# tbpaolini/PyJpegDecoder

Measured on AMD Instinct MI355X. Metric: megapixels/sec decoded (1080p 4:2:0 baseline batch), higher is better.
Workload: dtype f32; 1 GPU; 1024 x 1920x1080 4:2:0 baseline JPEG per GPU, q85, DRI=120 (one MCU row, 68 segments/image), on-GPU Huffman + dequant/IDCT/upsample/RGB (BASELINE configs[2]); images_per_gpu=1024, images_all_gpus=1024, distinct_images_per_gpu=256, layout=xmajor, restart_segmentation=host, entropy_bytes_per_image=667743

## Files before the change

pyjpegdecoder_amd/csrc/fused.hip:

```cpp
#include <stdio.h>
#include <string.h>

#include <algorithm>
#include <type_traits>
#include <vector>

#include "mijpeg_internal.h"
#include "lanes13_walk.h"
#include "reconstruct_fast_strips.h"

#pragma clang fp contract(off)

namespace mj {

namespace {

constexpr int kFusedLds = 160 * 1024;
constexpr int kFusedCtrl = 384;
constexpr int kFusedBitmap = 128;
constexpr int kFusedThreads = 1024;

struct FusedArgs {
    lanes13::Args L;
    ReconArgs R;
    const int64_t *job_prefix;
    int64_t total_jobs;
    int32_t jobs_per_image;
    int32_t n_prod, n_cons;
    int32_t ipw, n_pass, n_virt;
    int32_t spi;
    int32_t ri;
    int32_t n_images;
    int32_t pieces, piece_mcus, mcus_per_row, mcu_rows;
    int32_t col_pieces, piece_rows;
    int32_t simd_split;
    int32_t newest;
    uint32_t *x_counter;
    uint32_t *x_progress;
    const int32_t *x_holder;
    uint32_t *x_left;
    int32_t x_patience;
};

typedef uint32_t __attribute__((address_space(3))) *lds_word;
typedef uint32_t __attribute__((address_space(3))) *lds_word_t;

constexpr unsigned long long kFusedGuardTicks = 200000000ull;
__device__ __forceinline__ bool guard_expired(unsigned long long t0) { return __builtin_amdgcn_s_memrealtime() - t0 > kFusedGuardTicks; }

struct JobGeo {
    uint32_t ri, mpr, mcv, spi;
    uint32_t pieces, piece_mcus;
    uint32_t col_pieces, piece_rows;
};

template <bool BY_ROWS>
struct FusedSource {
    static constexpr bool kSingleJobs = true;
    uint32_t ctrl;
    uint32_t n_tickets;
    uint32_t v0, n_pass, ipp, n_images;
    uint32_t jobs_per_image, lpw;
    JobGeo g;
    int32_t *status;
    int lane;
    uint32_t newest, wpi, n_prod_w, pref;
    __device__ __forceinline__ uint32_t ctl_word(uint32_t addr) const {
        return (uint32_t)__builtin_amdgcn_readfirstlane((int)*(volatile uint32_t __attribute__((address_space(3))) *)(uintptr_t)addr);
    }
    __device__ __forceinline__ uint32_t claim() const {
        const uint32_t ih = images_in(0);
        for (;;) {
            const bool all_done = ctl_word(ctrl + 4u) >= n_prod_w;
            for (uint32_t jj = 0; jj < ih; ++jj) {
                const uint32_t j = pref + jj < ih ? pref + jj : pref + jj - ih;
                uint32_t r = g.mpr;
                if (!all_done) {
                    const uint32_t w0 = (j * g.spi) / lpw, w1 = (j * g.spi + g.spi - 1u) / lpw;
                    for (uint32_t w = w0; w <= w1; ++w) r = min(r, ctl_word(ctrl + 8u + 4u * w));
                }
                while (r > 0u) {
                    const uint32_t w = (r - 1u) >> 5, hi = r - (w << 5);
                    const uint32_t addr = ctrl + (uint32_t)kFusedBitmap + 4u * (j * wpi + w);
                    const uint32_t avail = ~ctl_word(addr) & (hi >= 32u ? 0xFFFFFFFFu : (1u << hi) - 1u);
                    if (avail == 0u) { r = w << 5; continue; }
                    const uint32_t b = 31u - (uint32_t)__builtin_clz(avail);
                    uint32_t old = 0;
                    if (lane == 0) old = __hip_atomic_fetch_or((lds_word_t)(uintptr_t)addr, 1u << b, __ATOMIC_RELAXED, __HIP_MEMORY_SCOPE_WORKGROUP);
                    old = (uint32_t)__builtin_amdgcn_readfirstlane((int)old);
                    if (!(old & (1u << b))) return (v0 * ipp + j) * jobs_per_image + (w << 5) + b;
                }
            }
            if (all_done) return ~0u;
            __builtin_amdgcn_s_sleep(8);
        }
    }
    __device__ __forceinline__ uint32_t images_in(uint32_t pass) const {
        const uint32_t lo = (v0 + pass) * ipp;
        return lo >= n_images ? 0u : min(ipp, n_images - lo);
    }
    __device__ __forceinline__ uint32_t draw() const {
        uint32_t t = 0;
        if (lane == 0) t = __hip_atomic_fetch_add((lds_word)(uintptr_t)ctrl, 1u, __ATOMIC_RELAXED, __HIP_MEMORY_SCOPE_WORKGROUP);
        return t;
    }
    __device__ __forceinline__ uint32_t take(uint32_t t) const { return (uint32_t)__builtin_amdgcn_readfirstlane((int)t); }
    __device__ __forceinline__ uint32_t first_job(uint32_t ticket) const {
        if constexpr (!BY_ROWS) { if (newest) return claim(); }
        uint32_t pass = 0, ih = images_in(0);
        for (; pass + 1 < n_pass; ++pass) {
            const uint32_t tp = ih * jobs_per_image;
            if (ticket < tp) break;
            ticket -= tp;
            ih = images_in(pass + 1);
        }
        const uint32_t img0 = (v0 + pass) * ipp;
        if constexpr (BY_ROWS) {
            const uint32_t rows = ih * g.mcv, pc = ticket / rows, rr = ticket - pc * rows, j = rr / g.mcv, row = rr - j * g.mcv;
            return (img0 + j) * jobs_per_image + row * g.pieces + pc;
        } else {
            const uint32_t m = ticket / ih, j = ticket - m * ih;
            return (img0 + j) * jobs_per_image + m;
        }
    }
    __device__ __forceinline__ uint32_t end_job(uint32_t ticket, uint32_t) const { return newest ? 0u : first_job(ticket) + 1u; }
    __device__ __forceinline__ uint32_t word(uint32_t j, uint32_t s) const {
        return *(volatile uint32_t __attribute__((address_space(3))) *)(uintptr_t)(ctrl + 8u + 4u * ((j * g.spi + s) / lpw));
    }
    __device__ __forceinline__ bool ready(uint32_t job) const {
        if (newest) return true;
        const uint32_t img = job / jobs_per_image, m = job - img * jobs_per_image, v = img / ipp, j = img - v * ipp;
        const uint32_t base = (v - v0) << kFusedPassShift;
        if constexpr (BY_ROWS) {
            const uint32_t row = m / g.pieces, pc = m - row * g.pieces, a = pc * g.piece_mcus, b = min(a + g.piece_mcus, g.mpr);
            const uint32_t g0 = row * g.mpr + a, g1 = row * g.mpr + b - 1u;
            bool ok = true;
            for (uint32_t s = g0 / g.ri; s <= g1 / g.ri; ++s) {
                const uint32_t need = min(g1, (s + 1u) * g.ri - 1u) - s * g.ri;
                ok = ok && (uint32_t)__builtin_amdgcn_readfirstlane((int)word(j, s)) > base + need;
            }
            return ok;
        }
        const uint32_t mc = m / g.col_pieces, q = m - mc * g.col_pieces, r_lo = q * g.piece_rows, r_hi = min(r_lo + g.piece_rows, g.mcv);
        if (g.ri == g.mpr) {
            const uint32_t w0 = (j * g.spi + r_lo) / lpw, w1 = (j * g.spi + r_hi - 1u) / lpw;
            uint32_t least = 0x7FFFFFFFu;
            for (uint32_t w = w0; w <= w1; ++w) {
                const uint32_t p = *(volatile uint32_t __attribute__((address_space(3))) *)(uintptr_t)(ctrl + 8u + 4u * w);
                least = min(least, p);
            }
            return (uint32_t)__builtin_amdgcn_readfirstlane((int)least) > base + mc;
        }
        bool behind = false;
        for (uint32_t r0 = r_lo; r0 < r_hi; r0 += 64u) {
            const uint32_t row = r0 + (uint32_t)lane;
            if (row < r_hi) {
                const uint32_t gi = row * g.mpr + mc, s = gi / g.ri;
                behind = behind || word(j, s) <= base + (gi - s * g.ri);
            }
        }
        return __builtin_amdgcn_ballot_w64(behind) == 0;
    }
    __device__ __forceinline__ bool wait_ready(uint32_t job) const {
        if (ready(job)) return true;
        const unsigned long long t0 = __builtin_amdgcn_s_memrealtime();
        while (!ready(job)) {
            __builtin_amdgcn_s_sleep(8);
            if (guard_expired(t0)) {
                if (lane == 0) atomicMax(status + job / jobs_per_image, MJ_ST_INTERNAL);
                break;
            }
        }
        return true;
    }
};

template <bool BY_ROWS>
struct FusedSourceX {
    static constexpr bool kSingleJobs = true;
    uint32_t *counter;
    const uint32_t *progress;
    const int32_t *holder;
    uint32_t n_tickets, n_images, jobs_per_image;
    JobGeo g;
    uint32_t *left_count, *left_list;
    uint32_t patience;
    int32_t *status;
    int lane;
    __device__ __forceinline__ uint32_t draw() const {
        uint32_t t = 0;
        if (lane == 0) t = __hip_atomic_fetch_add(counter, 1u, __ATOMIC_RELAXED, __HIP_MEMORY_SCOPE_AGENT);
        return t;
    }
    __device__ __forceinline__ uint32_t take(uint32_t t) const { return (uint32_t)__builtin_amdgcn_readfirstlane((int)t); }
    __device__ __forceinline__ uint32_t first_job(uint32_t ticket) const {
        if constexpr (BY_ROWS) {
            const uint32_t rows = n_images * g.mcv, pc = ticket / rows, rr = ticket - pc * rows, img = rr / g.mcv, row = rr - img * g.mcv;
            return img * jobs_per_image + row * g.pieces + pc;
        } else {
            const uint32_t m = ticket / n_images, img = ticket - m * n_images;
            return img * jobs_per_image + m;
        }
    }
    __device__ __forceinline__ uint32_t end_job(uint32_t ticket, uint32_t) const { return first_job(ticket) + 1u; }
    __device__ __forceinline__ uint32_t word(uint32_t img, uint32_t s) const {
        return __hip_atomic_load(progress + holder[img * g.spi + s], __ATOMIC_RELAXED, __HIP_MEMORY_SCOPE_AGENT);
    }
    __device__ __forceinline__ bool ready(uint32_t job) const {
        const uint32_t img = job / jobs_per_image, m = job - img * jobs_per_image;
        bool behind = false;
        if constexpr (BY_ROWS) {
            const uint32_t row = m / g.pieces, pc = m - row * g.pieces, a = pc * g.piece_mcus, b = min(a + g.piece_mcus, g.mpr);
// ... 3 lines not shown
            const uint32_t mc = m / g.col_pieces, q = m - mc * g.col_pieces, r_lo = q * g.piece_rows, r_hi = min(r_lo + g.piece_rows, g.mcv);
            for (uint32_t r0 = r_lo; r0 < r_hi; r0 += 64u) {
                const uint32_t row = r0 + (uint32_t)lane;
                if (row < r_hi) {
                    const uint32_t gi = row * g.mpr + mc, s = gi / g.ri;
                    behind = behind || word(img, s) <= gi - s * g.ri;
                }
            }
        }
        if (__builtin_amdgcn_ballot_w64(behind) != 0) return false;
        __builtin_amdgcn_fence(__ATOMIC_ACQUIRE, "agent");
        return true;
    }
    __device__ __forceinline__ bool wait_ready(uint32_t job) const {
        for (uint32_t spins = 0; !ready(job); ++spins) {
            __builtin_amdgcn_s_sleep(16);
            if (spins >= patience) {
                if (lane == 0) left_list[__hip_atomic_fetch_add(left_count, 1u, __ATOMIC_RELAXED, __HIP_MEMORY_SCOPE_AGENT)] = job;
                return false;
            }
        }
        return true;
    }
};

}

template <int HS, int VS, bool T, bool XWG>
__global__ __launch_bounds__(kFusedThreads) void k_fused(FusedArgs F) {
    using G = rfast::FGeo<HS, VS, 3>;
    extern __shared__ __attribute__((aligned(16))) unsigned char smem[];
    const int tid = threadIdx.x, lane = tid & 63;
    const int n_prod = F.n_prod, n_cons = F.n_cons;
    int wave = __builtin_amdgcn_readfirstlane(tid >> 6);
    if (F.simd_split) {
        const int simd = wave & 3, slot = wave >> 2, r = slot * 2 + (simd & 1);
        if (simd < 2) wave = r < n_prod ? r : n_prod + n_cons + (r - n_prod);
        else wave = r < n_cons ? n_prod + r : n_prod + n_cons + (8 - min(n_prod, 8)) + (r - n_cons);
        wave = min(wave, kFusedThreads / 64 - 1);
    }
    uint32_t *ctrl = reinterpret_cast<uint32_t *>(smem + kFusedLds - kFusedCtrl);
    float4 *wts = reinterpret_cast<float4 *>(smem + kFusedLds - kFusedCtrl - G::WTS_BYTES);
    if (tid < kFusedCtrl / 4) ctrl[tid] = 0;
    lanes13::stage<true>(F.L, smem, tid, kFusedThreads, n_prod);
    rfast::fill_weights<HS, VS, 3, T>(wts, tid, kFusedThreads);
    __syncthreads();

    typename std::conditional<XWG, FusedSourceX<T>, FusedSource<T>>::type src;
    const uint32_t ctrl_lds = lanes13::lds_addr(ctrl);
    const uint32_t v0 = (uint32_t)blockIdx.x * (uint32_t)F.n_pass;
    src.n_images = (uint32_t)F.n_images;
    src.jobs_per_image = (uint32_t)F.jobs_per_image;
    src.g = JobGeo{(uint32_t)F.ri, (uint32_t)F.mcus_per_row, (uint32_t)F.mcu_rows, (uint32_t)F.spi, (uint32_t)F.pieces, (uint32_t)F.piece_mcus,
                   (uint32_t)F.col_pieces, (uint32_t)F.piece_rows};
    if constexpr (XWG) {
        src.counter = F.x_counter; src.progress = F.x_progress; src.holder = F.x_holder;
        src.left_count = F.x_counter + 1; src.left_list = F.x_left; src.patience = (uint32_t)F.x_patience;
        src.n_tickets = src.n_images * src.jobs_per_image;
    } else {
        src.ctrl = ctrl_lds;
        src.v0 = v0; src.n_pass = (uint32_t)F.n_pass; src.ipp = (uint32_t)F.ipw;
        src.lpw = (uint32_t)F.L.lpw;
        src.newest = (uint32_t)F.newest; src.wpi = ((uint32_t)F.mcus_per_row + 31u) >> 5; src.n_prod_w = (uint32_t)n_prod;
        src.pref = (uint32_t)wave % max(1u, src.images_in(0));
        uint32_t mine = 0;
        for (uint32_t p = 0; p < src.n_pass; ++p) mine += src.images_in(p);
        src.n_tickets = mine * src.jobs_per_image;
    }
    src.lane = lane;
    src.status = F.L.status;

#ifdef MJ_DIAGNOSTIC
    unsigned long long *dbg = reinterpret_cast<unsigned long long *>(F.R.dump + (3u << 20)) + (size_t)(blockIdx.x & 1023) * 8;
    if (tid == 0) dbg[0] = __builtin_amdgcn_s_memrealtime();
#endif
    unsigned long long *clk = reinterpret_cast<unsigned long long *>(F.R.dump + kDumpClockWords);
    if (blockIdx.x == 0 && tid == 0) { clk[0] = __builtin_amdgcn_s_memtime(); clk[1] = __builtin_amdgcn_s_memrealtime(); }
    unsigned char *my_lds;
    if (wave < n_prod) {
        if constexpr (XWG) {
            lanes13::walk<2>(F.L, smem, lane, wave, n_prod, (int)blockIdx.x, (int)gridDim.x, lanes13::lds_addr(ctrl + 2 + wave));
        } else {
            for (int p = 0; p < F.n_pass && (int)v0 + p < F.n_virt; ++p)
                lanes13::walk<1>(F.L, smem, lane, wave, n_prod, (int)v0 + p, F.n_virt, lanes13::lds_addr(ctrl + 2 + wave), (uint32_t)p << kFusedPassShift);
        }
        __builtin_amdgcn_s_setprio(0);
#ifdef MJ_DIAGNOSTIC
        if (lane == 0) {
            const unsigned long long t = __builtin_amdgcn_s_memrealtime();
            atomicMin(dbg + 1, t);
            atomicMax(dbg + 2, t);
            if constexpr (!XWG) atomicMax(dbg + 4, (unsigned long long)*(volatile uint32_t __attribute__((address_space(3))) *)(uintptr_t)ctrl_lds);
        }
#endif
        if (lane == 0) __hip_atomic_fetch_add((lds_word)(uintptr_t)lanes13::lds_addr(ctrl + 1), 1u, __ATOMIC_RELEASE, __HIP_MEMORY_SCOPE_WORKGROUP);
    }
    if (wave >= n_prod && wave < n_prod + n_cons) {
        my_lds = smem + kFusedLds - kFusedCtrl - G::WTS_BYTES - (wave - n_prod + 1) * G::WAVE_BYTES;
    } else {
        {
            const unsigned long long t0 = __builtin_amdgcn_s_memrealtime();
            while ((int)*(volatile uint32_t __attribute__((address_space(3))) *)(uintptr_t)(ctrl_lds + 4u) < n_prod) {
                __builtin_amdgcn_s_sleep(16);
                if (guard_expired(t0)) return;
            }
        }
        __builtin_amdgcn_fence(__ATOMIC_ACQUIRE, "workgroup");
        const int k = wave < n_prod ? wave : wave - n_cons;
        if (k >= (int)((kFusedLds - kFusedCtrl - G::WTS_BYTES) / G::WAVE_BYTES) - n_cons) return;
        my_lds = smem + k * G::WAVE_BYTES;
    }
    rfast::strips_worker<HS, VS, 3, false, T>(F.R, F.job_prefix, F.total_jobs, F.jobs_per_image, my_lds, wts, lane, (int)blockIdx.x, wave, src);
    if (blockIdx.x == 0 && lane == 0) {
        atomicMax(clk + 2, (unsigned long long)__builtin_amdgcn_s_memtime());
        atomicMax(clk + 3, (unsigned long long)__builtin_amdgcn_s_memrealtime());
    }
#ifdef MJ_DIAGNOSTIC
    if (lane == 0) atomicMax(dbg + 3, (unsigned long long)__builtin_amdgcn_s_memrealtime());
#endif
}

#ifdef MJ_DIAGNOSTIC
void dbg_fused_report(const uint8_t *dump, int n_wg) {
    std::vector<unsigned long long> h((size_t)1024 * 8);
    (void)hipMemcpy(h.data(), dump + (3u << 20), h.size() * 8, hipMemcpyDeviceToHost);
    double first = 0, last = 0, end = 0, drawn = 0, end_max = 0;
    const int n = std::min(n_wg, 1024);
    unsigned long long t0 = ~0ull;
    for (int i = 0; i < n; ++i) t0 = std::min(t0, h[(size_t)i * 8]);
    for (int i = 0; i < n; ++i) {
        const unsigned long long *r = h.data() + (size_t)i * 8;
        first += (double)(r[1] - r[0]) * 0.01; last += (double)(r[2] - r[0]) * 0.01; end += (double)(r[3] - r[0]) * 0.01; drawn += (double)r[4];
        end_max = std::max(end_max, (double)(r[3] - t0) * 0.01);
    }
    fprintf(stderr, "[diag fused] %d workgroups; per workgroup (us from its start): first producer through %.0f, last %.0f, last wave out %.0f; tickets drawn when the "
                    "last producer was through %.0f; launch (first start to last end) %.0f us\n", n, first / n, last / n, end / n, drawn / n, end_max);
}
void dbg_fused_clear(uint8_t *dump) {
    std::vector<unsigned long long> z((size_t)1024 * 8, 0);
    for (size_t i = 0; i < 1024; ++i) z[i * 8 + 1] = ~0ull;
    (void)hipMemcpy(dump + (3u << 20), z.data(), z.size() * 8, hipMemcpyHostToDevice);
}
#endif


template <bool BY_ROWS>
struct LeftoverSource {
    static constexpr bool kSingleJobs = true;
    FusedSourceX<BY_ROWS> map;
    uint32_t *counter;
    const uint32_t *list;
    uint32_t n_left, first_undrawn, n_tickets;
    int lane;
    __device__ __forceinline__ uint32_t draw() const {
        uint32_t t = 0;
        if (lane == 0) t = __hip_atomic_fetch_add(counter, 1u, __ATOMIC_RELAXED, __HIP_MEMORY_SCOPE_AGENT);
        return t;
    }
    __device__ __forceinline__ uint32_t take(uint32_t t) const { return (uint32_t)__builtin_amdgcn_readfirstlane((int)t); }
    __device__ __forceinline__ uint32_t first_job(uint32_t ticket) const {
        return ticket < n_left ? list[ticket] : map.first_job(first_undrawn + (ticket - n_left));
    }
    __device__ __forceinline__ uint32_t end_job(uint32_t ticket, uint32_t) const { return first_job(ticket) + 1u; }
    __device__ __forceinline__ bool ready(uint32_t) const { return true; }
    __device__ __forceinline__ bool wait_ready(uint32_t) const { return true; }
};

template <int HS, int VS, bool T>
__global__ __launch_bounds__(256, 3) void k_recon_leftover(FusedArgs F) {
    using G = rfast::FGeo<HS, VS, 3>;
    extern __shared__ __attribute__((aligned(16))) unsigned char smem[];
    const uint32_t n_left = __hip_atomic_load(F.x_counter + 1, __ATOMIC_RELAXED, __HIP_MEMORY_SCOPE_AGENT);
    const uint32_t all = (uint32_t)F.n_images * (uint32_t)F.jobs_per_image;
    const uint32_t drawn = min(__hip_atomic_load(F.x_counter, __ATOMIC_RELAXED, __HIP_MEMORY_SCOPE_AGENT), all);
    if (n_left == 0 && drawn == all) return;
    const int tid = threadIdx.x, lane = tid & 63;
    const int wave = __builtin_amdgcn_readfirstlane(tid >> 6);
    if constexpr (G::SUB) {
        rfast::fill_weights<HS, VS, 3, T>(reinterpret_cast<float4 *>(smem + 4 * G::WAVE_BYTES), tid, 256);
        __syncthreads();
    }
// ... 72 lines not shown

extern "C" int mj_debug_fused_shape(int32_t cus, int32_t n_ac, int32_t n_dc, int32_t ac_slot_bytes, int32_t hmax, int32_t vmax, int32_t transposed,
                                    int32_t n_images, int32_t segments_per_image, int32_t want_consumers, int32_t out[8]) {
    if (!out) return MJ_ERR_INVALID;
    const mj::FusedShape s = mj::fused_shape(cus, n_ac * ac_slot_bytes, n_dc, hmax, vmax, transposed != 0, n_images, segments_per_image, want_consumers);
    out[0] = s.ok ? 1 : 0; out[1] = s.ipw; out[2] = s.n_prod; out[3] = s.lpw; out[4] = s.n_cons;
    out[5] = s.ok ? (int32_t)mj::lanes13::lds_bytes(s.ac_total_bytes, n_dc, s.n_prod, s.lpw, s.ring, s.dbits) : 0;
    out[6] = s.n_pass; out[7] = s.n_wg;
    return MJ_OK;
}

namespace mj {

hipError_t launch_fused(hipStream_t stream, const FusedShape &shape, const uint32_t *dstream, const int32_t *seg_bits, const DevSegment *segs,
                        int64_t n_segs, const DevImage *images, const DevHuff *huff, const uint16_t *lut11, const uint32_t *lut13,
                        int n_ac, int n_dc, uint64_t ac_slot_pk, uint64_t dc_slot_pk, uint64_t dc_tab_pk, const int ac_off[4], const int ac_bits[4],
                        int16_t *coef, int32_t *status,
                        const ReconArgs &a, int hmax, int vmax, bool transposed, int spi, int restart_interval, int mcus_per_row, int mcu_rows,
                        const int64_t *job_prefix, int64_t total_jobs, int jobs_per_image, const int32_t *by_length, const int32_t *holder,
                        uint32_t *x_words) {
    if (restart_interval < 1 || spi < 1) return hipErrorInvalidValue;
    if (!shape.ok || a.n_images < 1) return hipErrorInvalidValue;
    if (shape.xwg && (!by_length || !holder || !x_words)) return hipErrorInvalidValue;
    FusedArgs F{};
    F.L = lanes13::Args{dstream, seg_bits, segs, n_segs, images, huff, lut11, lut13, n_ac, n_dc, ac_slot_pk, dc_slot_pk, dc_tab_pk,
                        coef, status, shape.lpw, transposed ? 1 : 0, nullptr, nullptr, 0, shape.ring, shape.ac_total_bytes, shape.dbits,
                        {ac_off[0], ac_off[1], ac_off[2], ac_off[3]}, {ac_bits[0], ac_bits[1], ac_bits[2], ac_bits[3]}, shape.ipw * spi, nullptr};
    F.R = a;
    F.job_prefix = job_prefix; F.total_jobs = total_jobs; F.jobs_per_image = jobs_per_image;
    F.n_prod = shape.n_prod; F.n_cons = shape.n_cons; F.ipw = shape.ipw; F.n_pass = shape.n_pass; F.n_virt = shape.n_virt;
    F.spi = spi; F.ri = restart_interval; F.n_images = a.n_images;
    F.pieces = 1; F.piece_mcus = mcus_per_row; F.mcus_per_row = mcus_per_row; F.mcu_rows = mcu_rows;
    F.col_pieces = 1; F.piece_rows = mcu_rows;
    if (const char *e = opt("MJ_FUSED_SIMD_SPLIT")) F.simd_split = atoi(e) != 0 && shape.n_prod <= 8 && shape.n_cons <= 8;
    F.newest = !shape.xwg && !transposed && shape.n_pass == 1 && restart_interval == mcus_per_row && F.col_pieces == 1 &&
               shape.ipw * ((mcus_per_row + 31) / 32) <= (kFusedCtrl - kFusedBitmap) / 4;
    if (const char *e = opt("MJ_FUSED_ORDER")) F.newest = F.newest && !strcmp(e, "newest");
    else F.newest = 0;
    if (!transposed) {
        const int tmw = fast_tile_mcus(hmax, vmax, 3, false), spc = (mcu_rows + tmw - 1) / tmw;
        F.col_pieces = (spc + a.chunk_strips - 1) / a.chunk_strips;
        F.piece_rows = a.chunk_strips * tmw;
        if (jobs_per_image != mcus_per_row * F.col_pieces) return hipErrorInvalidValue;
    }
    if (transposed) {
        const int tmw = fast_tile_mcus(hmax, vmax, 3, true);
        int piece = 20;
        if (const char *e = opt("MJ_FUSED_PIECE")) piece = atoi(e);
        const int strips = std::max(1, piece / tmw);
        const int spc = (mcus_per_row + tmw - 1) / tmw;
        F.R.chunk_strips = strips;
        F.pieces = (spc + strips - 1) / strips;
        F.piece_mcus = strips * tmw;
        F.jobs_per_image = mcu_rows * F.pieces;
        F.total_jobs = (int64_t)a.n_images * F.jobs_per_image;
    }
    unsigned blocks = 0;
    if (shape.xwg) {
        const int64_t words = 32 + (int64_t)shape.n_wg * shape.n_prod;
        if (hipError_t e = launch_fill_words(stream, x_words, 0u, words); e != hipSuccess) return e;
        F.x_counter = x_words; F.x_progress = x_words + 32; F.x_holder = holder;
        F.x_left = x_words + 32 + (int64_t)shape.n_wg * shape.n_prod;
        F.x_patience = 2000;
        if (const char *e = opt("MJ_FUSED_PATIENCE")) F.x_patience = atoi(e);
        F.L.by_length = by_length; F.L.order_mode = 2; F.L.progress_global = F.x_progress;
        blocks = (unsigned)shape.n_wg;
    } else {
        blocks = (unsigned)shape.n_wg;
    }
    auto go = [&](auto kernel) {
        static OncePerDevice attr_once;
// ... 47 lines not shown
```

pyjpegdecoder_amd/csrc/options.hip:

```cpp
#include <string.h>
#include <stdlib.h>

#include <mutex>
#include <string>

#include "mijpeg_internal.h"

namespace mj {
namespace {
struct OptionRule { const char *name; const char *words; int lo, hi, step; };
const OptionRule kOptionRules[] = {
    {"MJ_HUFFMAN", "wave|lanes|lanes11|sync", 0, 0, 1}, {"MJ_SEG_ORDER", "blob|binned|striped", 0, 0, 1},
    {"MJ_SYNC_ROUNDS", nullptr, 0, 64, 1},   {"MJ_SYNC_CHUNK", nullptr, 256, 65536, 4}, {"MJ_SYNC_WARM", nullptr, 0, 65536, 1},
    {"MJ_PROG_BANDS", nullptr, 0, 1, 1},     {"MJ_PROG_ROWS", nullptr, 1, 4096, 1},     {"MJ_PROG_FAST", nullptr, 0, 1, 1},
    {"MJ_LANES_WAVES", nullptr, 1, 16, 1},   {"MJ_LANES_PER_WAVE", nullptr, 1, 64, 1},  {"MJ_LANES_RING", "64|128", 0, 0, 1},
    {"MJ_STAGE2_CHUNK", nullptr, 1, 4096, 1}, {"MJ_PROG_SPLIT", nullptr, 0, 3, 1},      {"MJ_PROG_PARTS", nullptr, 1, kProgSub, 1},
    {"MJ_FUSED", nullptr, 0, 1, 1},          {"MJ_FUSED_CONSUMERS", nullptr, 0, 15, 1},  {"MJ_FUSED_PATIENCE", nullptr, 0, 1000000, 1},
    {"MJ_FUSED_LUMA13", nullptr, 0, 1, 1},   {"MJ_SYNC_COUNT", "classic|resolved", 0, 0, 1}, {"MJ_SYNC_BITS", nullptr, 10, 13, 1},
    {"MJ_FUSED_ACBITS", nullptr, 10, 13, 1}, {"MJ_FUSED_PRODUCERS", nullptr, 1, 8, 1}, {"MJ_FUSED_SIMD_SPLIT", nullptr, 0, 1, 1}, {"MJ_FUSED_ORDER", "ticket|newest", 0, 0, 1},
    {"MJ_FUSED_PIECE", nullptr, 1, 4096, 1},
    {"MJ_PROG_CHUNKS", nullptr, 0, 2, 1},    {"MJ_PROG_CHUNK", nullptr, 128, 65536, 4},
};
constexpr int kNumOptions = (int)(sizeof(kOptionRules) / sizeof(kOptionRules[0]));
struct OptionTable {
    std::mutex mu;
    struct Entry { std::string value; bool set = false; };
    Entry e[kNumOptions];
};
OptionTable g_options;
bool option_value_ok(const OptionRule &r, const char *v) {
    if (r.words) {
        const size_t n = strlen(v);
        for (const char *w = r.words; *w;) {
            const char *bar = strchr(w, '|');
            const size_t len = bar ? (size_t)(bar - w) : strlen(w);
            if (len == n && !strncmp(w, v, n)) return true;
            w += len + (bar ? 1 : 0);
        }
        return false;
    }
    char *end = nullptr;
    const long x = strtol(v, &end, 10);
    return end != v && *end == 0 && x >= r.lo && x <= r.hi && x % r.step == 0;
}
}
const char *opt(const char *name) {
    thread_local std::string ring[8];
    thread_local unsigned turn = 0;
    {
        std::lock_guard<std::mutex> lk(g_options.mu);
        for (int i = 0; i < kNumOptions; ++i)
            if (!strcmp(kOptionRules[i].name, name)) {
// ... 49 lines not shown
```

pyjpegdecoder_amd/csrc/reconstruct_fast_strips.h:

```cpp
#pragma once
#include "mijpeg_internal.h"
#include "upsample_taps.h"

#pragma clang fp contract(off)

namespace mj {
namespace rfast {

#ifdef MJ_X_NTLOAD
typedef uint32_t mj_u32x4 __attribute__((ext_vector_type(4)));
__device__ __forceinline__ uint4 coef_load_nt(const uint4 *p) {
    const mj_u32x4 v = __builtin_nontemporal_load(reinterpret_cast<const mj_u32x4 *>(p));
    return make_uint4(v.x, v.y, v.z, v.w);
}
#define MJ_COEF_LOAD(p) coef_load_nt(p)
#else
#define MJ_COEF_LOAD(p) (*(p))
#endif

constexpr double kA = 0.35355339059327373;
constexpr double kC2 = 0.46193976625564337, kC6 = 0.19134171618254492;
constexpr double kC1 = 0.4903926402016152, kC3 = 0.4157348061512726, kC5 = 0.27778511650980114, kC7 = 0.09754516100806417;

__device__ __forceinline__ void idct8(const double f[8], double t[8]) {
// ... 197 lines not shown
}

static __device__ __noinline__ void block_exact(const int16_t *cblk, const uint16_t *qblk, const double *tt, int16_t *out_lds,
                                         int16_t *idct_out , bool transposed, bool chroma) {
    const int lane = threadIdx.x & 63;
    const int u = lane >> 3, v = lane & 7;
    const int src = transposed ? u * 8 + v : v * 8 + u;
    const int dn = deq(cblk[src], qblk[src]);
    const uint64_t mask = __ballot(dn != 0);
    double rsum[8];
#pragma unroll
    for (int vv = 0; vv < 8; ++vv) rsum[vv] = 0.0;
#pragma unroll 1
    for (int uu = 0; uu < 8; ++uu) {
        const uint32_t rowbits = (uint32_t)(mask >> (uu * 8)) & 0xFFu;
        if (rowbits == 0) continue;
#pragma unroll
        for (int vv = 0; vv < 8; ++vv) {
            if ((rowbits >> vv) & 1) {
                const int cc = __builtin_amdgcn_readlane(dn, uu * 8 + vv);
                const double p = (double)cc * tt[(uu * 8 + vv) * 64 + lane];
                rsum[vv] = rsum[vv] + p;
            }
        }
    }
    const double s = ((rsum[0] + rsum[1]) + (rsum[2] + rsum[3])) + ((rsum[4] + rsum[5]) + (rsum[6] + rsum[7]));
    const int raw = (int)(int16_t)(int)__builtin_rint(s), val = (int)(int16_t)(raw + 128);
    out_lds[transposed ? (lane & 7) * 8 + (lane >> 3) : lane] = (int16_t)(chroma ? raw : val);
    if (idct_out) idct_out[lane] = (int16_t)val;
}

struct TicketSource {
    static constexpr bool kSingleJobs = false;
    uint32_t *counter;
    uint32_t jpt, n_tickets, last_ticket;
    int lane;
    __device__ __forceinline__ uint32_t draw() const {
        uint32_t t = 0;
        if (lane == 0) t = __hip_atomic_fetch_add(counter, 1u, __ATOMIC_RELAXED, __HIP_MEMORY_SCOPE_AGENT);
        return t;
    }
    __device__ __forceinline__ uint32_t take(uint32_t t) const {
        const uint32_t c = (uint32_t)__builtin_amdgcn_readfirstlane((int)t);
        if (c == last_ticket && lane == 0) __hip_atomic_store(counter, 0u, __ATOMIC_RELAXED, __HIP_MEMORY_SCOPE_AGENT);
        return c;
    }
    __device__ __forceinline__ uint32_t first_job(uint32_t ticket) const { return ticket * jpt; }
    __device__ __forceinline__ uint32_t end_job(uint32_t ticket, uint32_t n_jobs) const { return min(n_jobs, (ticket + 1) * jpt); }
    __device__ __forceinline__ bool ready(uint32_t) const { return true; }
    __device__ __forceinline__ bool wait_ready(uint32_t) const { return true; }
};

template <int HS, int VS, int NC, bool T>
__device__ __forceinline__ void fill_weights(float4 *wt, int tid, int nthreads) {
    using G = FGeo<HS, VS, NC>;
    if constexpr (G::SUB) {
        constexpr float D = (float)kDen<HS, VS>;
        for (int i = tid; i < G::MW * G::MH; i += nthreads) {
            const uint32_t w = corner_weights<HS, VS, T>(i / G::MH, i % G::MH);
            wt[(i / G::MH) * G::WTS_ROW + (i % G::MH)] = make_float4((float)(w & 255) / D, (float)((w >> 8) & 255) / D, (float)((w >> 16) & 255) / D,
                                                                   (float)(w >> 24) / D);
        }
    }
}

template <int HS, int VS, int NC, bool SEAMS, bool T, class Src>
__device__ __forceinline__ void strips_worker(const ReconArgs &a, const int64_t *__restrict__ job_prefix, const int64_t total_jobs, const int jobs_per_image,
                                              unsigned char *wave_lds, const float4 *s_wts, const int lane, const int dump_slot, const int wave_in_wg, Src &src) {
    using G = FGeo<HS, VS, NC>;
    int16_t *s_strip = reinterpret_cast<int16_t *>(wave_lds);
    double *scr = reinterpret_cast<double *>(wave_lds + G::STRIP_BYTES) + (lane >> 3) * 72;
    float *scrf = reinterpret_cast<float *>(wave_lds + G::STRIP_BYTES) + (lane >> 3) * 124;
    uint16_t *s_qt = reinterpret_cast<uint16_t *>(wave_lds + G::STRIP_BYTES + G::SCR_BYTES);
    const int grp = lane >> 3, j = lane & 7;

    const int px = lane / G::TML, pk0 = lane % G::TML;

    struct Job {
        const DevImage *im;
        const int16_t *cfirst;
        int row_elems;
        int mcu_x, y_first, n_strips, mcv;
    };
    auto job_of = [&](uint32_t jb) -> Job {
        uint32_t img, r;
        if (a.uniform_geometry) {
            img = jb / (uint32_t)jobs_per_image;
            r = jb - img * (uint32_t)jobs_per_image;
        } else {
            int lo = 0, hi = a.n_images;
            while (hi - lo > 1) {
                int mid = (lo + hi) >> 1;
                if (job_prefix[mid] <= (int64_t)jb) lo = mid; else hi = mid;
            }
            img = (uint32_t)lo;
            r = jb - (uint32_t)job_prefix[lo];
        }
        img = (uint32_t)__builtin_amdgcn_readfirstlane((int)img);
        r = (uint32_t)__builtin_amdgcn_readfirstlane((int)r);
        Job jo;
        jo.im = a.images + img;
        const int mch = T ? cimg(jo.im)->mcu_count_v : cimg(jo.im)->mcu_count_h, mcv = T ? cimg(jo.im)->mcu_count_h : cimg(jo.im)->mcu_count_v;
        const uint32_t spc = (uint32_t)(mcv + G::TMW - 1) / G::TMW;
        const uint32_t S = (uint32_t)a.chunk_strips, pieces = (spc + S - 1) / S;
        jo.mcv = mcv;
        jo.mcu_x = __builtin_amdgcn_readfirstlane((int)(r / pieces));
        const uint32_t s0 = (r - (uint32_t)jo.mcu_x * pieces) * S;
        jo.n_strips = (int)min(S, spc - s0);
        jo.y_first = (int)s0 * G::TMW;
        if constexpr (T) {
            jo.row_elems = G::NB * 64;
            jo.cfirst = a.coef + (cimg(jo.im)->block_off + (int64_t)jo.mcu_x * mcv * G::NB) * 64 + (int64_t)jo.y_first * jo.row_elems;
        } else {
            jo.row_elems = mch * G::NB * 64;
            jo.cfirst = a.coef + (cimg(jo.im)->block_off + (int64_t)jo.mcu_x * G::NB) * 64 + (int64_t)jo.y_first * jo.row_elems;
        }
        return jo;
    };
    auto fetch_first = [&](const Job &jo, uint4 (&cw)[G::ROUNDS]) {
        const int nv = min(G::TMW, jo.mcv - jo.y_first);
#pragma unroll
        for (int r = 0; r < G::ROUNDS; ++r) {
            const int bt = min(r * 8 + grp, G::NBT - 1);
            const int k = bt / G::NB, b = bt - k * G::NB;
#ifdef MJ_X_SPARSE_LD
            if (NC == 3 && b >= G::NBY && j >= 4) cw[r] = MJ_COEF_LOAD(reinterpret_cast<const uint4 *>(a.dump + kDumpZeroLine));
            else
#endif
            cw[r] = MJ_COEF_LOAD(reinterpret_cast<const uint4 *>(jo.cfirst + __mul24(k < nv ? k : 0, jo.row_elems) + b * 64 + j * 8));
            asm volatile("" ::: "memory");
        }
    };

#ifdef MJ_DIAGNOSTIC
    const int dm = a.debug_mask;
    if (dm & 1) for (int i = lane; i < G::STRIP_BYTES / 2; i += 64) s_strip[i] = 0;
    if (a.debug == 12 && wave_in_wg >= 2) { for (int i = 0; i < 64; ++i) __builtin_amdgcn_s_sleep(127); }
    if (a.debug == 13 && (wave_in_wg & 1)) { for (int i = 0; i < 64; ++i) __builtin_amdgcn_s_sleep(127); }
    const uint64_t dbg_t0 = __builtin_amdgcn_s_memtime(), dbg_r0 = __builtin_amdgcn_s_memrealtime();
    uint64_t dbg_wait = 0, dbg_acc[6] = {0, 0, 0, 0, 0, 0}, dbg_last = dbg_t0;
#define MJ_STAMP(i) do { if (a.debug == 10) { uint64_t s_; asm volatile("s_memtime %0\n\ts_waitcnt lgkmcnt(0)" : "=s"(s_) :: "memory"); dbg_acc[i] += s_ - dbg_last; dbg_last = s_; } } while (0)
#endif
    const uint32_t n_jobs = (uint32_t)total_jobs;
    uint32_t ticket = src.take(src.draw());
    if (ticket >= src.n_tickets) return;
    uint32_t job = src.first_job(ticket);
    if (job >= n_jobs) return;
    const DevImage *qt_owner = nullptr;
    uint4 cw[G::ROUNDS];
  for (;;) {
    if (!src.wait_ready(job)) return;
    fetch_first(job_of(job), cw);
    bool stalled = false;
    if constexpr (!SEAMS) {
        constexpr int NT0 = (G::MW * G::TMW * G::MH * NC / 16 + 63) / 64;
        unsigned char *dump0 = a.dump + ((size_t)(dump_slot & 4095) * 64 + lane) * 16;
#pragma unroll
        for (int t = 0; t < NT0; ++t) *reinterpret_cast<volatile u32x4_a4 *>(dump0) = u32x4_a4{0u, 0u, 0u, (uint32_t)t};
    }
    for (;;) {
      const uint32_t ticket_v = src.draw();
      const uint32_t job_end = src.end_job(ticket, n_jobs);
      for (;;) {
        const Job jo = job_of(job);
        const DevImage *im_g = jo.im;
        const ConstImage im = cimg(im_g);
        const int W = T ? im->height : im->width, H = T ? im->width : im->height;
        const int mch_o = im->mcu_count_h;
        const int mcv_k = jo.mcv;
        const int mcu_x = jo.mcu_x;
        const int row_elems = jo.row_elems;
        const int64_t block_off = im->block_off;
        const uint16_t *qbase = a.qt;
        const int q0i = im->qt_index[0] * 64, q1i = im->qt_index[NC == 3 ? 1 : 0] * 64, q2i = im->qt_index[NC == 3 ? 2 : 0] * 64;
        if (im_g != qt_owner) {
            qt_owner = im_g;
            const int c = lane >> 4, part = lane & 15;
            if (c < 3) {
                const int qi = c == 0 ? q0i : (c == 1 ? q1i : q2i);
                reinterpret_cast<uint2 *>(s_qt)[c * 16 + part] = reinterpret_cast<const uint2 *>(qbase + qi)[part];
            }
        }
        const uint32_t n_strips = (uint32_t)jo.n_strips;
        uint32_t voff[G::ROUNDS];
#pragma unroll
        for (int r = 0; r < G::ROUNDS; ++r) {
            const int bt = min(r * 8 + grp, G::NBT - 1);
            const int k = bt / G::NB, b = bt - k * G::NB;
            voff[r] = (uint32_t)(__mul24(k, row_elems) + b * 64 + j * 8) * 2u;
        }
        const int16_t *cptr = jo.cfirst;
        int y_first = jo.y_first;
        const int64_t rgb_off = im->rgb_off;
        const int hnc_i = H * NC;
        unsigned char *const col_dst = a.rgb + rgb_off + (int64_t)(mcu_x * G::MW) * hnc_i;
      for (uint32_t si = 0;; ++si) {
        const int n_valid = min(G::TMW, mcv_k - y_first);
        auto mcu_block = [&](int k) -> int64_t {
            return block_off + (T ? (int64_t)(mcu_x * mch_o + y_first + k) : (int64_t)((y_first + k) * mch_o + mcu_x)) * G::NB;
        };

#ifdef MJ_DIAGNOSTIC
        MJ_STAMP(5);
        if (a.debug == 8 || a.debug == 9) {
            uint64_t s0, s1;
            asm volatile("s_memtime %0\n\ts_waitcnt lgkmcnt(0)" : "=s"(s0) :: "memory");
            if (a.debug == 8) asm volatile("s_waitcnt vmcnt(3)" ::: "memory"); else asm volatile("s_waitcnt vmcnt(0)" ::: "memory");
            asm volatile("s_memtime %0\n\ts_waitcnt lgkmcnt(0)" : "=s"(s1) :: "memory");
            dbg_wait += s1 - s0;
        }
// ... 183 lines not shown
            constexpr int NBYTES = G::MH * NC;
            unsigned char *const s_out = wave_lds + G::STRIP_BYTES;
            uint32_t ob[(NBYTES + 3) / 4];
            constexpr int RGB = G::MH / 8;
            int act_m = 0, slow_m = 0, rg_m = 0;
#pragma unroll
          for (int sv = 0; sv < G::SV; ++sv) {
            const int pk = pk0 + sv * G::TML;
#ifdef MJ_DIAGNOSTIC
            const bool have = pk < n_valid && a.debug != 2 && !(dm & 2);
#else
            const bool have = pk < n_valid;
#endif
            const int gx = mcu_x * G::MW + px, gy0 = (y_first + pk) * G::MH;
            const int16_t *mt = s_strip + pk * G::MCU_STRIDE;
            const int nrows = min(G::MH, H - gy0);
            unsigned char *dst = col_dst + (int64_t)px * hnc_i + gy0 * NC;

            if constexpr (SEAMS) {
                if (have && gx < W)
                    pixel_run_exact<HS, VS, NC, T>(mt, px, dst, nrows,
                                                   a.planes ? a.planes + (im->pix_off + (T ? (int64_t)gy0 * W + gx : (int64_t)gx * H + gy0)) * NC : nullptr,
                                                   T ? W * NC : NC);
            } else {
#pragma unroll
                for (int i = 0; i < (NBYTES + 3) / 4; ++i) ob[i] = 0;
                bool slow = false;
                int rg = 0;
                if (have) {
                if constexpr (NC == 3) {
                    const int sx0 = src_pos<HS>(px);
                    const int sx1 = sx0 < 7 ? sx0 + 1 : 7;
                    const int16_t *cbp = mt + G::NBY * 64, *crp = cbp + 64;
                    const uint4 ba = *reinterpret_cast<const uint4 *>(cbp + sx0 * 8), ra = *reinterpret_cast<const uint4 *>(crp + sx0 * 8);
                    const uint32_t bw[4] = {ba.x, ba.y, ba.z, ba.w}, rw[4] = {ra.x, ra.y, ra.z, ra.w};
                    uint32_t bw2[4] = {0, 0, 0, 0}, rw2[4] = {0, 0, 0, 0};
                    if constexpr (HS > 1) {
                        const uint4 bb = *reinterpret_cast<const uint4 *>(cbp + sx1 * 8), rb = *reinterpret_cast<const uint4 *>(crp + sx1 * 8);
                        bw2[0] = bb.x; bw2[1] = bb.y; bw2[2] = bb.z; bw2[3] = bb.w;
                        rw2[0] = rb.x; rw2[1] = rb.y; rw2[2] = rb.z; rw2[3] = rb.w;
                    }
                    auto pairA = [&](int i) { return f32x2{(float)((i & 1) ? hi16(bw[i >> 1]) : lo16(bw[i >> 1])), (float)((i & 1) ? hi16(rw[i >> 1]) : lo16(rw[i >> 1]))}; };
                    auto pairB = [&](int i) { return f32x2{(float)((i & 1) ? hi16(bw2[i >> 1]) : lo16(bw2[i >> 1])), (float)((i & 1) ? hi16(rw2[i >> 1]) : lo16(rw2[i >> 1]))}; };
                    float crange = 0.0f;
                    bool tie125;
                    {
                        typedef short s16x2 __attribute__((ext_vector_type(2)));
                        auto pmax = [](uint32_t a, uint32_t b) { return __builtin_bit_cast(uint32_t, __builtin_elementwise_max(__builtin_bit_cast(s16x2, a), __builtin_bit_cast(s16x2, b))); };
                        auto pmin = [](uint32_t a, uint32_t b) { return __builtin_bit_cast(uint32_t, __builtin_elementwise_min(__builtin_bit_cast(s16x2, a), __builtin_bit_cast(s16x2, b))); };
                        uint32_t mx = pmax(pmax(bw[0], bw[1]), pmax(bw[2], bw[3])), mn = pmin(pmin(bw[0], bw[1]), pmin(bw[2], bw[3]));
                        if constexpr (HS > 1) {
                            mx = pmax(mx, pmax(pmax(bw2[0], bw2[1]), pmax(bw2[2], bw2[3])));
                            mn = pmin(mn, pmin(pmin(bw2[0], bw2[1]), pmin(bw2[2], bw2[3])));
                        }
                        const int hi_ = max(lo16(mx), hi16(mx)), lo_ = min(lo16(mn), hi16(mn));
                        tie125 = !((hi_ < 125 && lo_ > -125) || lo_ > 125 || hi_ < -125);
                    }
                    constexpr float MAGIC = 12582912.0f;
#pragma unroll
                    for (int by = 0; by < G::MH / 8; ++by) {
                        const int yb = T ? (px >> 3) * VS + by : by * HS + (px >> 3);
                        const uint4 yw = *reinterpret_cast<const uint4 *>(mt + yb * 64 + (px & 7) * 8);
                        const uint32_t ywd[4] = {yw.x, yw.y, yw.z, yw.w};
                        const int s_lo = (G::SUB && VS > 1) ? src_pos<VS>(by * 8) : 0;
                        f32x2 cA[8], cB[8];
#pragma unroll
                        for (int i = 0; i < 8; ++i) {
                            const bool used = !G::SUB || VS == 1 || (i >= s_lo && i <= src_pos<VS>(by * 8 + 7) + 1);
                            if (used) {
                                cA[i] = pairA(i);
                                crange = __builtin_fmaxf(__builtin_fmaxf(__builtin_fabsf(cA[i].x), __builtin_fabsf(cA[i].y)), crange);
                                if constexpr (HS > 1) {
                                    cB[i] = pairB(i);
                                    crange = __builtin_fmaxf(__builtin_fmaxf(__builtin_fabsf(cB[i].x), __builtin_fabsf(cB[i].y)), crange);
                                }
                            }
                        }
                        auto chroma_of = [&](int i) -> f32x2 {
                            if constexpr (G::SUB) {
                                const int y = by * 8 + i;
                                const int sy0 = src_pos<VS>(y);
                                const int sy1 = sy0 < 7 ? sy0 + 1 : 7;
                                const float4 wq = s_wts[px * G::WTS_ROW + y];
                                f32x2 sv = cA[sy0] * wq.x;
                                sv = __builtin_elementwise_fma(cA[sy1], f32x2{wq.y, wq.y}, sv);
                                if constexpr (HS > 1) {
                                    sv = __builtin_elementwise_fma(cB[sy0], f32x2{wq.z, wq.z}, sv);
                                    sv = __builtin_elementwise_fma(cB[sy1], f32x2{wq.w, wq.w}, sv);
                                }
                                return f32x2{__builtin_rintf(sv.x), __builtin_rintf(sv.y)};
                            } else {
                                return cA[i];
                            }
// ... 191 lines not shown
```

Baseline: 354,700 MP/s.

## Remove newest-order claiming and SIMD split, tune register pressure in fused reconstruct

Removes the optional 'newest' bitmap-claim scheduling and SIMD-split wave remapping, which were off by default, along with their options. Adds a compile-time kUniform flag so fused sources skip the non-uniform geometry lookup. Inserts asm barriers on lane values and a zero register to stop the compiler from hoisting or rematerialising address math. Reloads the chroma source words from LDS on each luma block row instead of keeping them live across the loop. These register-pressure tweaks aim to lower VGPR use in the hot reconstruct loop, at the cost of extra LDS reads.

After: 357,200 MP/s (median of 6 runs). Within noise of the previous version (+0.7%).

```diff
diff --git a/pyjpegdecoder_amd/csrc/fused.hip b/pyjpegdecoder_amd/csrc/fused.hip
--- a/pyjpegdecoder_amd/csrc/fused.hip
+++ b/pyjpegdecoder_amd/csrc/fused.hip
@@ -17,7 +17,6 @@
 
 constexpr int kFusedLds = 160 * 1024;
 constexpr int kFusedCtrl = 384;
-constexpr int kFusedBitmap = 128;
 constexpr int kFusedThreads = 1024;
 
 struct FusedArgs {
@@ -33,8 +32,6 @@
     int32_t n_images;
     int32_t pieces, piece_mcus, mcus_per_row, mcu_rows;
     int32_t col_pieces, piece_rows;
-    int32_t simd_split;
-    int32_t newest;
     uint32_t *x_counter;
     uint32_t *x_progress;
     const int32_t *x_holder;
@@ -43,7 +40,6 @@
 };
 
 typedef uint32_t __attribute__((address_space(3))) *lds_word;
-typedef uint32_t __attribute__((address_space(3))) *lds_word_t;
 
 constexpr unsigned long long kFusedGuardTicks = 200000000ull;
 __device__ __forceinline__ bool guard_expired(unsigned long long t0) { return __builtin_amdgcn_s_memrealtime() - t0 > kFusedGuardTicks; }
@@ -57,6 +53,7 @@
 template <bool BY_ROWS>
 struct FusedSource {
     static constexpr bool kSingleJobs = true;
+    static constexpr bool kUniform = true;
     uint32_t ctrl;
     uint32_t n_tickets;
     uint32_t v0, n_pass, ipp, n_images;
@@ -64,37 +61,6 @@
     JobGeo g;
     int32_t *status;
     int lane;
-    uint32_t newest, wpi, n_prod_w, pref;
-    __device__ __forceinline__ uint32_t ctl_word(uint32_t addr) const {
-        return (uint32_t)__builtin_amdgcn_readfirstlane((int)*(volatile uint32_t __attribute__((address_space(3))) *)(uintptr_t)addr);
-    }
-    __device__ __forceinline__ uint32_t claim() const {
-        const uint32_t ih = images_in(0);
-        for (;;) {
-            const bool all_done = ctl_word(ctrl + 4u) >= n_prod_w;
-            for (uint32_t jj = 0; jj < ih; ++jj) {
-                const uint32_t j = pref + jj < ih ? pref + jj : pref + jj - ih;
-                uint32_t r = g.mpr;
-                if (!all_done) {
-                    const uint32_t w0 = (j * g.spi) / lpw, w1 = (j * g.spi + g.spi - 1u) / lpw;
-                    for (uint32_t w = w0; w <= w1; ++w) r = min(r, ctl_word(ctrl + 8u + 4u * w));
-                }
-                while (r > 0u) {
-                    const uint32_t w = (r - 1u) >> 5, hi = r - (w << 5);
-                    const uint32_t addr = ctrl + (uint32_t)kFusedBitmap + 4u * (j * wpi + w);
-                    const uint32_t avail = ~ctl_word(addr) & (hi >= 32u ? 0xFFFFFFFFu : (1u << hi) - 1u);
-                    if (avail == 0u) { r = w << 5; continue; }
-                    const uint32_t b = 31u - (uint32_t)__builtin_clz(avail);
-                    uint32_t old = 0;
-                    if (lane == 0) old = __hip_atomic_fetch_or((lds_word_t)(uintptr_t)addr, 1u << b, __ATOMIC_RELAXED, __HIP_MEMORY_SCOPE_WORKGROUP);
-                    old = (uint32_t)__builtin_amdgcn_readfirstlane((int)old);
-                    if (!(old & (1u << b))) return (v0 * ipp + j) * jobs_per_image + (w << 5) + b;
-                }
-            }
-            if (all_done) return ~0u;
-            __builtin_amdgcn_s_sleep(8);
-        }
-    }
     __device__ __forceinline__ uint32_t images_in(uint32_t pass) const {
         const uint32_t lo = (v0 + pass) * ipp;
         return lo >= n_images ? 0u : min(ipp, n_images - lo);
@@ -106,7 +72,6 @@
     }
     __device__ __forceinline__ uint32_t take(uint32_t t) const { return (uint32_t)__builtin_amdgcn_readfirstlane((int)t); }
     __device__ __forceinline__ uint32_t first_job(uint32_t ticket) const {
-        if constexpr (!BY_ROWS) { if (newest) return claim(); }
         uint32_t pass = 0, ih = images_in(0);
         for (; pass + 1 < n_pass; ++pass) {
             const uint32_t tp = ih * jobs_per_image;
@@ -123,12 +88,11 @@
             return (img0 + j) * jobs_per_image + m;
         }
     }
-    __device__ __forceinline__ uint32_t end_job(uint32_t ticket, uint32_t) const { return newest ? 0u : first_job(ticket) + 1u; }
+    __device__ __forceinline__ uint32_t end_job(uint32_t ticket, uint32_t) const { return first_job(ticket) + 1u; }
     __device__ __forceinline__ uint32_t word(uint32_t j, uint32_t s) const {
         return *(volatile uint32_t __attribute__((address_space(3))) *)(uintptr_t)(ctrl + 8u + 4u * ((j * g.spi + s) / lpw));
     }
     __device__ __forceinline__ bool ready(uint32_t job) const {
-        if (newest) return true;
         const uint32_t img = job / jobs_per_image, m = job - img * jobs_per_image, v = img / ipp, j = img - v * ipp;
         const uint32_t base = (v - v0) << kFusedPassShift;
         if constexpr (BY_ROWS) {
@@ -178,6 +142,7 @@
 template <bool BY_ROWS>
 struct FusedSourceX {
     static constexpr bool kSingleJobs = true;
+    static constexpr bool kUniform = true;
     uint32_t *counter;
     const uint32_t *progress;
     const int32_t *holder;
@@ -247,13 +212,7 @@
     extern __shared__ __attribute__((aligned(16))) unsigned char smem[];
     const int tid = threadIdx.x, lane = tid & 63;
     const int n_prod = F.n_prod, n_cons = F.n_cons;
-    int wave = __builtin_amdgcn_readfirstlane(tid >> 6);
-    if (F.simd_split) {
-        const int simd = wave & 3, slot = wave >> 2, r = slot * 2 + (simd & 1);
-        if (simd < 2) wave = r < n_prod ? r : n_prod + n_cons + (r - n_prod);
-        else wave = r < n_cons ? n_prod + r : n_prod + n_cons + (8 - min(n_prod, 8)) + (r - n_cons);
-        wave = min(wave, kFusedThreads / 64 - 1);
-    }
+    const int wave = __builtin_amdgcn_readfirstlane(tid >> 6);
     uint32_t *ctrl = reinterpret_cast<uint32_t *>(smem + kFusedLds - kFusedCtrl);
     float4 *wts = reinterpret_cast<float4 *>(smem + kFusedLds - kFusedCtrl - G::WTS_BYTES);
     if (tid < kFusedCtrl / 4) ctrl[tid] = 0;
@@ -276,8 +235,6 @@
         src.ctrl = ctrl_lds;
         src.v0 = v0; src.n_pass = (uint32_t)F.n_pass; src.ipp = (uint32_t)F.ipw;
         src.lpw = (uint32_t)F.L.lpw;
-        src.newest = (uint32_t)F.newest; src.wpi = ((uint32_t)F.mcus_per_row + 31u) >> 5; src.n_prod_w = (uint32_t)n_prod;
-        src.pref = (uint32_t)wave % max(1u, src.images_in(0));
         uint32_t mine = 0;
         for (uint32_t p = 0; p < src.n_pass; ++p) mine += src.images_in(p);
         src.n_tickets = mine * src.jobs_per_image;
@@ -296,8 +253,11 @@
         if constexpr (XWG) {
             lanes13::walk<2>(F.L, smem, lane, wave, n_prod, (int)blockIdx.x, (int)gridDim.x, lanes13::lds_addr(ctrl + 2 + wave));
         } else {
-            for (int p = 0; p < F.n_pass && (int)v0 + p < F.n_virt; ++p)
-                lanes13::walk<1>(F.L, smem, lane, wave, n_prod, (int)v0 + p, F.n_virt, lanes13::lds_addr(ctrl + 2 + wave), (uint32_t)p << kFusedPassShift);
+            for (int p = 0; p < F.n_pass && (int)v0 + p < F.n_virt; ++p) {
+                int lane_p = lane;
+                asm volatile("" : "+v"(lane_p));
+                lanes13::walk<1>(F.L, smem, lane_p, wave, n_prod, (int)v0 + p, F.n_virt, lanes13::lds_addr(ctrl + 2 + wave), (uint32_t)p << kFusedPassShift);
+            }
         }
         __builtin_amdgcn_s_setprio(0);
 #ifdef MJ_DIAGNOSTIC
@@ -362,6 +322,7 @@
 template <bool BY_ROWS>
 struct LeftoverSource {
     static constexpr bool kSingleJobs = true;
+    static constexpr bool kUniform = true;
     FusedSourceX<BY_ROWS> map;
     uint32_t *counter;
     const uint32_t *list;
@@ -500,11 +461,6 @@
     F.spi = spi; F.ri = restart_interval; F.n_images = a.n_images;
     F.pieces = 1; F.piece_mcus = mcus_per_row; F.mcus_per_row = mcus_per_row; F.mcu_rows = mcu_rows;
     F.col_pieces = 1; F.piece_rows = mcu_rows;
-    if (const char *e = opt("MJ_FUSED_SIMD_SPLIT")) F.simd_split = atoi(e) != 0 && shape.n_prod <= 8 && shape.n_cons <= 8;
-    F.newest = !shape.xwg && !transposed && shape.n_pass == 1 && restart_interval == mcus_per_row && F.col_pieces == 1 &&
-               shape.ipw * ((mcus_per_row + 31) / 32) <= (kFusedCtrl - kFusedBitmap) / 4;
-    if (const char *e = opt("MJ_FUSED_ORDER")) F.newest = F.newest && !strcmp(e, "newest");
-    else F.newest = 0;
     if (!transposed) {
         const int tmw = fast_tile_mcus(hmax, vmax, 3, false), spc = (mcu_rows + tmw - 1) / tmw;
         F.col_pieces = (spc + a.chunk_strips - 1) / a.chunk_strips;
diff --git a/pyjpegdecoder_amd/csrc/options.hip b/pyjpegdecoder_amd/csrc/options.hip
--- a/pyjpegdecoder_amd/csrc/options.hip
+++ b/pyjpegdecoder_amd/csrc/options.hip
@@ -17,7 +17,7 @@
     {"MJ_STAGE2_CHUNK", nullptr, 1, 4096, 1}, {"MJ_PROG_SPLIT", nullptr, 0, 3, 1},      {"MJ_PROG_PARTS", nullptr, 1, kProgSub, 1},
     {"MJ_FUSED", nullptr, 0, 1, 1},          {"MJ_FUSED_CONSUMERS", nullptr, 0, 15, 1},  {"MJ_FUSED_PATIENCE", nullptr, 0, 1000000, 1},
     {"MJ_FUSED_LUMA13", nullptr, 0, 1, 1},   {"MJ_SYNC_COUNT", "classic|resolved", 0, 0, 1}, {"MJ_SYNC_BITS", nullptr, 10, 13, 1},
-    {"MJ_FUSED_ACBITS", nullptr, 10, 13, 1}, {"MJ_FUSED_PRODUCERS", nullptr, 1, 8, 1}, {"MJ_FUSED_SIMD_SPLIT", nullptr, 0, 1, 1}, {"MJ_FUSED_ORDER", "ticket|newest", 0, 0, 1},
+    {"MJ_FUSED_ACBITS", nullptr, 10, 13, 1}, {"MJ_FUSED_PRODUCERS", nullptr, 1, 8, 1},
     {"MJ_FUSED_PIECE", nullptr, 1, 4096, 1},
     {"MJ_PROG_CHUNKS", nullptr, 0, 2, 1},    {"MJ_PROG_CHUNK", nullptr, 128, 65536, 4},
 };
diff --git a/pyjpegdecoder_amd/csrc/reconstruct_fast_strips.h b/pyjpegdecoder_amd/csrc/reconstruct_fast_strips.h
--- a/pyjpegdecoder_amd/csrc/reconstruct_fast_strips.h
+++ b/pyjpegdecoder_amd/csrc/reconstruct_fast_strips.h
@@ -253,6 +253,7 @@
 
 struct TicketSource {
     static constexpr bool kSingleJobs = false;
+    static constexpr bool kUniform = false;
     uint32_t *counter;
     uint32_t jpt, n_tickets, last_ticket;
     int lane;
@@ -305,7 +306,7 @@
     };
     auto job_of = [&](uint32_t jb) -> Job {
         uint32_t img, r;
-        if (a.uniform_geometry) {
+        if (Src::kUniform || a.uniform_geometry) {
             img = jb / (uint32_t)jobs_per_image;
             r = jb - img * (uint32_t)jobs_per_image;
         } else {
@@ -340,6 +341,9 @@
     };
     auto fetch_first = [&](const Job &jo, uint4 (&cw)[G::ROUNDS]) {
         const int nv = min(G::TMW, jo.mcv - jo.y_first);
+        int lane_f = lane;
+        asm volatile("" : "+v"(lane_f));
+        const int grp = lane_f >> 3, j = lane_f & 7;
 #pragma unroll
         for (int r = 0; r < G::ROUNDS; ++r) {
             const int bt = min(r * 8 + grp, G::NBT - 1);
@@ -348,7 +352,8 @@
             if (NC == 3 && b >= G::NBY && j >= 4) cw[r] = MJ_COEF_LOAD(reinterpret_cast<const uint4 *>(a.dump + kDumpZeroLine));
             else
 #endif
-            cw[r] = MJ_COEF_LOAD(reinterpret_cast<const uint4 *>(jo.cfirst + __mul24(k < nv ? k : 0, jo.row_elems) + b * 64 + j * 8));
+            const uint32_t off = (uint32_t)(__mul24(k < nv ? k : 0, jo.row_elems) + b * 64 + j * 8) * 2u;
+            cw[r] = MJ_COEF_LOAD(reinterpret_cast<const uint4 *>(reinterpret_cast<const unsigned char *>(jo.cfirst) + off));
             asm volatile("" ::: "memory");
         }
     };
@@ -375,9 +380,11 @@
     bool stalled = false;
     if constexpr (!SEAMS) {
         constexpr int NT0 = (G::MW * G::TMW * G::MH * NC / 16 + 63) / 64;
-        unsigned char *dump0 = a.dump + ((size_t)(dump_slot & 4095) * 64 + lane) * 16;
-#pragma unroll
-        for (int t = 0; t < NT0; ++t) *reinterpret_cast<volatile u32x4_a4 *>(dump0) = u32x4_a4{0u, 0u, 0u, (uint32_t)t};
+        uint32_t zero = 0u;
+        asm volatile("" : "+v"(zero));
+        unsigned char *dump0 = a.dump + (size_t)(dump_slot & 4095) * 1024 + ((uint32_t)lane + zero) * 16u;
+#pragma unroll
+        for (int t = 0; t < NT0; ++t) *reinterpret_cast<volatile u32x4_a4 *>(dump0) = u32x4_a4{zero, zero, zero, zero + (uint32_t)t};
     }
     for (;;) {
       const uint32_t ticket_v = src.draw();
@@ -396,7 +403,9 @@
         const int q0i = im->qt_index[0] * 64, q1i = im->qt_index[NC == 3 ? 1 : 0] * 64, q2i = im->qt_index[NC == 3 ? 2 : 0] * 64;
         if (im_g != qt_owner) {
             qt_owner = im_g;
-            const int c = lane >> 4, part = lane & 15;
+            int lane_q = lane;
+            asm volatile("" : "+v"(lane_q));
+            const int c = lane_q >> 4, part = lane_q & 15;
             if (c < 3) {
                 const int qi = c == 0 ? q0i : (c == 1 ? q1i : q2i);
                 reinterpret_cast<uint2 *>(s_qt)[c * 16 + part] = reinterpret_cast<const uint2 *>(qbase + qi)[part];
@@ -646,14 +655,18 @@
                     const int sx0 = src_pos<HS>(px);
                     const int sx1 = sx0 < 7 ? sx0 + 1 : 7;
                     const int16_t *cbp = mt + G::NBY * 64, *crp = cbp + 64;
-                    const uint4 ba = *reinterpret_cast<const uint4 *>(cbp + sx0 * 8), ra = *reinterpret_cast<const uint4 *>(crp + sx0 * 8);
-                    const uint32_t bw[4] = {ba.x, ba.y, ba.z, ba.w}, rw[4] = {ra.x, ra.y, ra.z, ra.w};
-                    uint32_t bw2[4] = {0, 0, 0, 0}, rw2[4] = {0, 0, 0, 0};
-                    if constexpr (HS > 1) {
-                        const uint4 bb = *reinterpret_cast<const uint4 *>(cbp + sx1 * 8), rb = *reinterpret_cast<const uint4 *>(crp + sx1 * 8);
-                        bw2[0] = bb.x; bw2[1] = bb.y; bw2[2] = bb.z; bw2[3] = bb.w;
-                        rw2[0] = rb.x; rw2[1] = rb.y; rw2[2] = rb.z; rw2[3] = rb.w;
-                    }
+                    uint32_t bw[4], rw[4], bw2[4] = {0, 0, 0, 0}, rw2[4] = {0, 0, 0, 0};
+                    auto read_src = [&]() {
+                        const uint4 ba = *reinterpret_cast<const uint4 *>(cbp + sx0 * 8), ra = *reinterpret_cast<const uint4 *>(crp + sx0 * 8);
+                        bw[0] = ba.x; bw[1] = ba.y; bw[2] = ba.z; bw[3] = ba.w;
+                        rw[0] = ra.x; rw[1] = ra.y; rw[2] = ra.z; rw[3] = ra.w;
+                        if constexpr (HS > 1) {
+                            const uint4 bb = *reinterpret_cast<const uint4 *>(cbp + sx1 * 8), rb = *reinterpret_cast<const uint4 *>(crp + sx1 * 8);
+                            bw2[0] = bb.x; bw2[1] = bb.y; bw2[2] = bb.z; bw2[3] = bb.w;
+                            rw2[0] = rb.x; rw2[1] = rb.y; rw2[2] = rb.z; rw2[3] = rb.w;
+                        }
+                    };
+                    read_src();
                     auto pairA = [&](int i) { return f32x2{(float)((i & 1) ? hi16(bw[i >> 1]) : lo16(bw[i >> 1])), (float)((i & 1) ? hi16(rw[i >> 1]) : lo16(rw[i >> 1]))}; };
                     auto pairB = [&](int i) { return f32x2{(float)((i & 1) ? hi16(bw2[i >> 1]) : lo16(bw2[i >> 1])), (float)((i & 1) ? hi16(rw2[i >> 1]) : lo16(rw2[i >> 1]))}; };
                     float crange = 0.0f;
@@ -673,6 +686,10 @@
                     constexpr float MAGIC = 12582912.0f;
 #pragma unroll
                     for (int by = 0; by < G::MH / 8; ++by) {
+                        if (by > 0) {
+                            asm volatile("" ::: "memory");
+                            read_src();
+                        }
                         const int yb = T ? (px >> 3) * VS + by : by * HS + (px >> 3);
                         const uint4 yw = *reinterpret_cast<const uint4 *>(mt + yb * 64 + (px & 7) * 8);
                         const uint32_t ywd[4] = {yw.x, yw.y, yw.z, yw.w};
```
